# CSU-KangHu/HiTE

Hardware: AMD Instinct MI355X
Metric: candidate TE boundaries/sec on 1 Gbp synthetic genome (fine stage: copy finding+gather+align+vote+judge) (higher is better)
Workload: dtype u8; 1 GPU; C3: 1000 Mbp synthetic genome, 2500 TIR + 2500 LTR families, 50000 candidates/GPU judged as TIR (copy finding by minimizer-index lookup inside the timed step; index build 0.0 s untimed); genome_bp=1000000000, candidates_per_gpu=50000, candidate_bases=192511237, copies=799813, copy_table=found, is_te=34225, parallelism=replicated genome, candidates per rank x1, all-gather of 32-B calls

## Files before the change

### hite_amd/_lib.py

```python
import ctypes as C
import os

import numpy as np

_HERE = os.path.dirname(os.path.abspath(__file__))
SO_PATH = os.path.join(_HERE, "libhite_gpu.so")

HITE_TE = {"tir": 0, "helitron": 1, "non_ltr": 2}
INFO = {0: "", 1: "nb", 2: "fl1", 3: "EXC"}
HITE_SUBCLUSTER_CHUNK = 64


class HiteError(RuntimeError):
    pass


class HiteCall(C.Structure):
    _fields_ = [("is_te", C.c_int32), ("info", C.c_int32), ("row_num", C.c_int32), ("bstart", C.c_int32),
                ("bend", C.c_int32), ("cons_len", C.c_int32), ("cons_off", C.c_int64)]


CALL_DTYPE = np.dtype([("is_te", "<i4"), ("info", "<i4"), ("row_num", "<i4"), ("bstart", "<i4"), ("bend", "<i4"),
                       ("cons_len", "<i4"), ("cons_off", "<i8")])
assert CALL_DTYPE.itemsize == 32 and C.sizeof(HiteCall) == 32
LCV_DTYPE = np.dtype([("body", "<u8"), ("care", "<u8"), ("gap_min", "u1"), ("gap_max", "u1"), ("body_len", "u1"), ("pad", "u1", (5,))])
assert LCV_DTYPE.itemsize == 24
HELITRON_MAX_BODY, HELITRON_MAX_GAP = 32, 63

_lib = None


def load():
    global _lib
    if _lib is None:
        if not os.path.exists(SO_PATH):
            raise HiteError("libhite_gpu.so not built: run `python -c 'import __graft_entry__ as g; g.build()'` "
                            "(or make -C hite_amd/csrc); there is no CPU fallback")
        lib = C.CDLL(SO_PATH)
        lib.hite_last_error.restype = C.c_char_p
        lib.hite_genome_bases.restype = C.c_int64
        lib.hite_host_free.restype = None
        lib.hite_host_free.argtypes = [C.c_void_p]
        lib.hite_protein_lib_release.restype = None
        lib.hite_protein_lib_release.argtypes = [C.c_void_p]
        _lib = lib
    return _lib


def _p(a):
    return a.ctypes.data_as(C.c_void_p) if a is not None else None


def _arr(x, dtype):
    return np.ascontiguousarray(x, dtype=dtype)


def seed_sub_shard(rank, world, s, S):
    if world <= 1:
        rank, world = 0, 1
    return rank * S + s, world * S


class Context:

    def __init__(self, device=0):
        self.lib = load()
        h = C.c_void_p()
        rc = self.lib.hite_ctx_create(int(device), C.byref(h))
        if rc != 0:
            raise HiteError("hite_ctx_create(device=%d) failed: %d (no usable GPU?)" % (device, rc))
        self.h = h
        self.device = device

    def copy_config(self, aligned_interval):
        self._check(self.lib.hite_copy_config_ctx(self.h, -1 if aligned_interval is None else int(bool(aligned_interval))), "hite_copy_config_ctx")

    def release_copy_index(self):
        if getattr(self, "_copy_state", None) is not None and getattr(self, "h", None):
            self.lib.hite_copy_index_release(self._copy_state)
        self._copy_state = None

    def close(self):
        self.release_copy_index()
        for lib in list(getattr(self, "_prot_libs", ())):
            lib.release()
        if getattr(self, "_pipe_state", None) is not None and getattr(self, "h", None):
            self.lib.hite_pipeline_release(self._pipe_state)
            self._pipe_state = C.c_void_p(None)
        if getattr(self, "h", None):
            self.lib.hite_ctx_destroy(self.h)
            self.h = None

    def __del__(self):
        try:
            self.close()
        except Exception:
            pass

    def _check(self, rc, what):
        if rc != 0:
            msg = self.lib.hite_last_error(self.h)
            raise HiteError("%s failed: %d %s" % (what, rc, (msg or b"").decode(errors="replace")))

    def genome_pack(self, seqs):
        bs = [s.encode() if isinstance(s, str) else bytes(s) for s in seqs]
        off = np.zeros(len(bs) + 1, dtype=np.int64)
        np.cumsum([len(b) for b in bs], out=off[1:])
        buf = np.frombuffer(b"".join(bs), dtype=np.uint8)
        self._check(self.lib.hite_genome_pack(self.h, _p(buf), _p(off), len(bs)), "hite_genome_pack")
        self.contig_len = np.diff(off)

    def set_contig_order(self, names):
        if names is None:
            self._check(self.lib.hite_set_contig_order(self.h, None, 0), "hite_set_contig_order")
            return
        keyed = sorted(range(len(names)), key=lambda i: (names[i] + ":").encode())
        rank = np.zeros(len(names), dtype=np.int32)
        rank[keyed] = np.arange(len(names), dtype=np.int32)
        self._check(self.lib.hite_set_contig_order(self.h, _p(rank), len(names)), "hite_set_contig_order")

    def genome_pack_dev(self, d_ptr, contig_off, stream=0):
        off = _arr(contig_off, np.int64)
        self._check(self.lib.hite_genome_pack_dev(self.h, C.c_void_p(d_ptr), _p(off), len(off) - 1, C.c_void_p(stream)),
                    "hite_genome_pack_dev")
        self.contig_len = np.diff(off)

    def flank_gather(self, contig, start1, end1, minus, flank=50):
        n = len(contig)
# ... 926 lines not shown
```

### hite_amd/csrc/hite_common.h

```cpp
#pragma once
#include <hip/hip_runtime.h>
#include <stdint.h>
#include <stdio.h>
#include <string.h>
#include <stdlib.h>
#include "../../include/hite_gpu.h"

#define HITE_WAVE 64
#define HITE_BLOCK 256

#define JUDGE_CLS_BLOCK 0
#define JUDGE_CLS_WAVE 1
#define JUDGE_CLS_LDS 2
#define JUDGE_LDS_WAVE_SIZES 3
#define JUDGE_LDS_BLOCK_SIZES 2
#define JUDGE_NCLS (JUDGE_CLS_LDS + JUDGE_LDS_WAVE_SIZES + JUDGE_LDS_BLOCK_SIZES)
#define HITE_AUX_STREAMS (JUDGE_NCLS - 1)
struct JudgeFuse {
    const uint8_t *win;
    const int64_t *win_off;
    const int32_t *win_len;
    const int32_t *row_first;
    const int64_t *ops_base;
    const uint16_t *ops;
    const uint32_t *lay;
    const int32_t *last_extra;
    const int32_t *row_map;
    const int32_t *rows_eff;
};

struct hite_ctx {
    int device;
    char err[512];
    uint32_t *d_bases;
    uint32_t *d_nmask;
    int64_t *d_contig_off;
    int64_t *h_contig_off;
    int32_t n_contigs;
    int64_t n_bases;
    int64_t genome_epoch;
    int64_t *mask_log;
    int64_t mask_log_n, mask_log_cap;
    void *d_scratch;
    size_t scratch_bytes;
    void *d_scratch2;
    size_t scratch2_bytes;
    int prof_on;
    int prof_n;
    char prof_name[64][32];
    double prof_ms[64];
    int64_t prof_count[64];
    int prof_pending;
    void *prof_ev[512][2];
    int prof_stage[512];
    void *align_state;
    const int32_t *d_msa_row_map;
    const int32_t *d_msa_rows_eff;
    uint32_t *d_msa_lay;
    int msa_long;
    const int64_t *d_msa_win_off;
    const int32_t *d_msa_win_len;
    const uint32_t *d_msa_pads;
    int32_t copy_interval;
    int32_t *d_contig_rank;
    void *aux_stream[HITE_AUX_STREAMS];
    void *aux_fork;
    void *aux_join[HITE_AUX_STREAMS];
    int32_t seed_rank, seed_world;
    const uint8_t *d_judge_cls;
    JudgeFuse judge_fuse;
    void *fmea_arena;
    int32_t subcluster_chunk;
    int64_t subcluster_batch_bytes;
    int64_t framecluster_batch_bytes;
    int64_t pairhsp_batch_pairs;
    int64_t ltrscan_batch_bytes;
};
void hite_fmea_release(hite_ctx *ctx);
int hite_aux_streams(hite_ctx *ctx, int k, hipStream_t *st, hipEvent_t *fork_ev, hipEvent_t *join_ev);

int hite_prof_begin(hite_ctx *ctx, const char *name, hipStream_t st);
void hite_prof_end(hite_ctx *ctx, int token, hipStream_t st);
void hite_prof_resolve(hite_ctx *ctx);

#define HITE_CHECK(ctx, call)                                                                         \
    do {                                                                                              \
        hipError_t e__ = (call);                                                                      \
        if (e__ != hipSuccess) {                                                                      \
            if (ctx) snprintf((ctx)->err, sizeof((ctx)->err), "%s:%d %s: %s", __FILE__, __LINE__, #call, \
                              hipGetErrorString(e__));                                                \
            return HITE_EHIP;                                                                         \
        }                                                                                             \
    } while (0)

int hite_scratch_reserve(hite_ctx *ctx, size_t bytes, void **out);
int hite_scratch2_reserve(hite_ctx *ctx, size_t bytes, void **out);

__device__ __forceinline__ int lane_id() { return threadIdx.x & 63; }
__device__ __forceinline__ int wave_id() { return threadIdx.x >> 6; }

__device__ __forceinline__ int sym_class(uint8_t c) {
    switch (c) {
        case 'A': return 0;
        case 'C': return 1;
        case 'G': return 2;
        case 'T': return 3;
        case '-': return 5;
        default: return 4;
    }
}
__device__ __forceinline__ uint8_t class_sym(int k) { return (uint8_t)("ACGTN-"[k]); }
__device__ __forceinline__ uint8_t fold_sym(uint8_t c) { return class_sym(sym_class(c)); }
// ... 44 lines not shown
```

### hite_amd/csrc/hite_ctx.hip

```cpp
#include "hite_common.h"
#include "hite_hostbuf.h"
#include "hite_align.h"
#include "hite_genome.h"

extern "C" int hite_version(void) { return 1; }

extern "C" int hite_ctx_create(int device_id, hite_ctx **out) {
    if (!out) return HITE_EINVAL;
    int ndev = 0;
    if (hipGetDeviceCount(&ndev) != hipSuccess || ndev <= 0) return HITE_ENODEV;
    if (device_id < 0 || device_id >= ndev) return HITE_EINVAL;
    hite_ctx *c = (hite_ctx *)calloc(1, sizeof(hite_ctx));
    if (!c) return HITE_ENOMEM;
    c->device = device_id;
    c->copy_interval = -1;
    c->subcluster_chunk = HITE_SUBCLUSTER_CHUNK;
    if (const char *e = getenv("HITE_SUBCLUSTER_CHUNK_ROWS")) {
        const long v = strtol(e, nullptr, 10);
        if (v >= 1 && v <= HITE_SUBCLUSTER_CHUNK) c->subcluster_chunk = (int32_t)v;
    }
    if (const char *e = getenv("HITE_SUBCLUSTER_BATCH_BYTES")) {
        const long long v = strtoll(e, nullptr, 10);
        if (v >= 1) c->subcluster_batch_bytes = (int64_t)v;
    }
    if (const char *e = getenv("HITE_FRAMECLUSTER_BATCH_BYTES")) {
        const long long v = strtoll(e, nullptr, 10);
        if (v >= 1 && v <= ((long long)1 << 30)) c->framecluster_batch_bytes = (int64_t)v;
    }
    if (const char *e = getenv("HITE_PAIRHSP_BATCH_PAIRS")) {
        const long long v = strtoll(e, nullptr, 10);
        if (v >= 1 && v <= ((long long)1 << 24)) c->pairhsp_batch_pairs = (int64_t)v;
    }
    if (const char *e = getenv("HITE_LTRSCAN_BATCH_BYTES")) {
        const long long v = strtoll(e, nullptr, 10);
        if (v >= 1 && v <= ((long long)1 << 30)) c->ltrscan_batch_bytes = (int64_t)v;
    }
    if (hipSetDevice(device_id) != hipSuccess) { free(c); return HITE_EHIP; }
    *out = c;
    return HITE_OK;
}

static void free_genome(hite_ctx *c) {
    if (c->d_contig_rank) { (void)hipFree(c->d_contig_rank); c->d_contig_rank = nullptr; }
    if (c->d_bases) (void)hipFree(c->d_bases);
    if (c->d_nmask) (void)hipFree(c->d_nmask);
    if (c->d_contig_off) (void)hipFree(c->d_contig_off);
    free(c->h_contig_off);
    c->d_bases = c->d_nmask = nullptr;
    c->d_contig_off = nullptr;
    c->h_contig_off = nullptr;
    c->n_contigs = 0;
    c->n_bases = 0;
    c->genome_epoch++;
    c->mask_log_n = 0;
}

extern "C" void hite_ctx_destroy(hite_ctx *c) {
    if (!c) return;
    (void)hipSetDevice(c->device);
    free_genome(c);
    free(c->mask_log);
    hite_align_release(c);
    hite_fmea_release(c);
    if (c->d_scratch) (void)hipFree(c->d_scratch);
    if (c->d_scratch2) (void)hipFree(c->d_scratch2);
    if (c->d_contig_rank) (void)hipFree(c->d_contig_rank);
    if (c->aux_fork) (void)hipEventDestroy((hipEvent_t)c->aux_fork);
    for (int i = 0; i < HITE_AUX_STREAMS; i++) {
// ... 421 lines not shown
```

### hite_amd/csrc/hite_msa.hip

```cpp
#include "hite_common.h"
#include "hite_hostbuf.h"
#include "hite_align.h"
#include "hite_scan.h"
#include "hite_fill.h"

#define MSA_MAXR 128

struct MsaParams {
    int n;
    int64_t total_rows;
    const uint8_t *win;
    const int64_t *win_off;
    const int32_t *win_len;
    const int32_t *row_first;
    const int64_t *ops_base;
    uint16_t *ops;
    int32_t *cols_out;
    int32_t *status;
    const int32_t *row_map;
    const int32_t *rows_eff;
    const uint32_t *pads;
    uint32_t *lay;
};

__device__ __forceinline__ int msa_rows(const int32_t *__restrict__ rows_eff, const int32_t *__restrict__ row_first, int c) {
    return rows_eff ? rows_eff[c] : row_first[c + 1] - row_first[c];
}
__device__ __forceinline__ int msa_src(const int32_t *__restrict__ row_map, int64_t g0, int r) {
    return row_map ? row_map[g0 + r] - (int)g0 : r;
}

__device__ __forceinline__ int row_ins_s(const uint16_t *__restrict__ rop, int p, int m, int nrow, int start) {
    int prev_end = start;
    if (p > 0) { unsigned o = rop[p - 1]; prev_end = (int)(o & 0x7fff) + ((o >> 15) ? 0 : 1); }
    int q = p < m ? (int)(rop[p] & 0x7fff) : nrow;
    return q - prev_end;
}
__device__ __forceinline__ int row_ins(const uint16_t *__restrict__ rop, int p, int m, int nrow) {
    const unsigned o = rop[p - 1];
    const int prev_end = (int)(o & 0x7fff) + ((o >> 15) ? 0 : 1);
    int q = p < m ? (int)(rop[p] & 0x7fff) : nrow;
    return q - prev_end;
}

__global__ void __launch_bounds__(256) star_layout_kernel(MsaParams P) {
    __shared__ int s_scan[8];
    const int c = blockIdx.x;
    if (c >= P.n) return;
    const int64_t g0 = P.row_first[c];
    const int R = msa_rows(P.rows_eff, P.row_first, c);
    if (R <= 0) { if (threadIdx.x == 0) P.cols_out[c] = 0; return; }
    const int m = P.win_len[g0];
    uint16_t *ops = P.ops + P.ops_base[c];
    uint16_t *insmax = ops;
    uint16_t *bstart = ops + (int64_t)R * (m + 1);
    if (P.status[c]) { if (threadIdx.x == 0) P.cols_out[c] = 0; return; }
    int running = 0;
// ... 246 lines not shown
    }
};
template <int NU>
__global__ void __launch_bounds__(256) star_fill_sparse_kernel(FillSparseParams Q) {
    const FillParams &P = Q.F;
    const int c = blockIdx.x;
    if (c >= P.n) return;
    const int C = P.cols[c];
    if (C <= 0 || (Q.cls && Q.cls[c] >= JUDGE_CLS_LDS)) return;
    const int64_t g0 = P.row_first[c];
    const int R = msa_rows(P.rows_eff, P.row_first, c);
    const int m = P.win_len[g0];
    const uint16_t *ops = P.ops + P.ops_base[c];
    const uint32_t *lay = Q.lay + (P.ops_base[c] >> 1);
    const int le = Q.last_extra[c];
    uint8_t *out = P.msa + P.msa_off[c];
    const int rs = m + 1;
    int r = blockIdx.y;
    if (r >= R) return;
    __shared__ unsigned s_defer[FILL_DEFER_CAP];
    __shared__ int s_ndefer;
    if (threadIdx.x == 0) s_ndefer = 0;
    __syncthreads();
    const bool can_defer = R <= 0xffff && m < 0xffff;
    int src = msa_src(P.row_map, g0, r);
    int64_t woff = P.win_off[g0 + src];
    int nrow = P.win_len[g0 + src];
    while (r < R) {
        const int rn = r + (int)gridDim.y;
        int64_t woff_n = 0; int nrow_n = 0;
        if (rn < R) { const int sn = msa_src(P.row_map, g0, rn); woff_n = P.win_off[g0 + sn]; nrow_n = P.win_len[g0 + sn]; }
        const uint8_t *b = P.win + woff;
        const uint16_t *rop = ops + (int64_t)r * rs;
        uint8_t *row = out + (int64_t)r * C;
        if (can_defer) fill_sparse_row<uint8_t *, 256, NU, FillDefer>(row, b, nrow, rop, lay, m, le, r == 0 , (int)threadIdx.x,
                                                                      FillDefer{s_defer, &s_ndefer, (unsigned)r});
        else fill_sparse_row<uint8_t *, 256, NU>(row, b, nrow, rop, lay, m, le, r == 0, (int)threadIdx.x);
        r = rn; woff = woff_n; nrow = nrow_n;
    }
    __syncthreads();
    const int nd = s_ndefer < FILL_DEFER_CAP ? s_ndefer : FILL_DEFER_CAP;
    for (int i = threadIdx.x; i < nd; i += 256) {
        const int rr = (int)(s_defer[i] >> 16), p = (int)(s_defer[i] & 0xffffu);
        const int sr = msa_src(P.row_map, g0, rr);
        const uint8_t *b = P.win + P.win_off[g0 + sr];
        const int nr = P.win_len[g0 + sr];
        const uint16_t *rop = ops + (int64_t)rr * rs;
        const unsigned w = lay[p];
        const unsigned oc = rr == 0 ? (unsigned)p : (p < m ? (unsigned)rop[p] : 0x8000u);
        fill_sparse_block<uint8_t *>(out + (int64_t)rr * C, b, nr, rop, m, le, rr == 0, p, w, oc);
    }
}

__global__ void __launch_bounds__(256) msa_compact_rows_kernel(int n, const int32_t *__restrict__ row_first,
                                                               const int32_t *__restrict__ win_len, const int64_t *__restrict__ ops_base,
                                                               uint16_t *__restrict__ ops_all, const int32_t *__restrict__ cand_flag,
                                                               const int32_t *__restrict__ row_dead, int32_t *__restrict__ row_map,
                                                               int32_t *__restrict__ rows_eff) {
    const int c = blockIdx.x;
    if (c >= n) return;
    const int g0 = row_first[c], R = row_first[c + 1] - g0;
    if (R <= 0) { if (threadIdx.x == 0) rows_eff[c] = 0; return; }
    if (cand_flag[c] != 2) {
        for (int r = threadIdx.x; r < R; r += 256) row_map[g0 + r] = g0 + r;
        if (threadIdx.x == 0) rows_eff[c] = R;
        return;
    }
    const int m = win_len[g0];
    uint16_t *ops = ops_all + ops_base[c];
    int k = 0;
    for (int r = 0; r < R; r++) {
        if (row_dead[g0 + r]) continue;
        if (k != r) for (int p = threadIdx.x; p <= m; p += 256) ops[(int64_t)k * (m + 1) + p] = ops[(int64_t)r * (m + 1) + p];
        if (threadIdx.x == 0) row_map[g0 + k] = g0 + r;
        k++;
        __syncthreads();
    }
    if (threadIdx.x == 0) rows_eff[c] = k;
}
__global__ void msa_rows_out_kernel(int n, const int32_t *__restrict__ row_first, const int32_t *__restrict__ rows_eff,
                                    int32_t *__restrict__ rows_out) {
    const int c = blockIdx.x * blockDim.x + threadIdx.x;
    if (c < n) rows_out[c] = rows_eff ? rows_eff[c] : row_first[c + 1] - row_first[c];
}

__global__ void row_pad_scan_kernel(int64_t total_rows, const uint8_t *__restrict__ win, const int64_t *__restrict__ win_off,
                                    const int32_t *__restrict__ win_len, int32_t *__restrict__ len2, uint32_t *__restrict__ pads) {
    const int64_t g = (int64_t)blockIdx.x * blockDim.x + threadIdx.x;
    if (g >= total_rows) return;
    const uint8_t *b = win + win_off[g];
    const int n = win_len[g];
    int pf = 0, pb = 0;
    if (n > 0 && HITE_IS_ROW_PAD(b[0])) { pf = 1; while (pf < n && HITE_IS_ROW_PAD(b[pf])) pf++; }
    if (pf < n && HITE_IS_ROW_PAD(b[n - 1])) { pb = 1; while (pf + pb < n && HITE_IS_ROW_PAD(b[n - 1 - pb])) pb++; }
    len2[g] = n - pb;
    pads[g] = (uint32_t)pf | ((uint32_t)pb << 16);
}
__global__ void __launch_bounds__(256) ops_pad_fix_kernel(int n, const int32_t *__restrict__ row_first, const int32_t *__restrict__ win_len,
                                                          const int64_t *__restrict__ ops_base, uint16_t *__restrict__ ops_all,
                                                          const uint32_t *__restrict__ pads, const int32_t *__restrict__ row_map,
                                                          const int32_t *__restrict__ rows_eff, int32_t *__restrict__ len2) {
    const int c = blockIdx.x;
    if (c >= n) return;
    const int g0 = row_first[c];
    const int R = rows_eff ? rows_eff[c] : row_first[c + 1] - g0;
    if (R >= 1 && threadIdx.x == 0) len2[g0] = win_len[g0];
// ... 8 lines not shown
        uint16_t *o = ops + (int64_t)k * (m + 1);
        if (lane == 0) o[-1] = (uint16_t)(0x8000u | (unsigned)pf);
        if (pf) {
            for (int base = 0; base < m; base += 64) {
                const int p = base + lane;
                const bool hit = p < m && (int)(o[p < m ? p : 0] & 0x7fffu) < pf;
                if (hit) o[p] = (uint16_t)(0x8000u | (unsigned)pf);
                if (__ballot(hit) != ~0ull) break;
            }
        }
        if (pb) {
            for (int top = m; top > 0; top -= 64) {
                const int p = top - 1 - lane;
                const bool hit = p >= 0 && (int)(o[p >= 0 ? p : 0] & 0x7fffu) >= hi;
                if (hit) o[p] = (uint16_t)(0x8000u | (unsigned)hi);
                if (__ballot(hit) != ~0ull) break;
            }
        }
    }
}

static int star_msa_launch(hite_ctx *ctx, int32_t n, const uint8_t *d_win, const int64_t *d_win_off,
                           const int32_t *d_win_len, const int32_t *d_row_first, int64_t total_rows, const int64_t *d_ops_base,
                           int64_t ops_elems, int32_t max_win_len, int32_t *d_cols_out, int32_t *d_status,
                           int32_t *d_new_cols, int32_t *d_last_extra, int32_t *d_rows_out, int32_t *d_info, void *stream) {
    if (!ctx || n < 0 || total_rows < 0 || max_win_len <= 0 || max_win_len > 32767) return HITE_EINVAL;
    if (n == 0) return HITE_OK;
    const size_t ops_bytes = ((size_t)ops_elems * 2 + 255) & ~(size_t)255;
    const size_t rows_bytes = ((size_t)total_rows * 4 + 255) & ~(size_t)255, cand_bytes = ((size_t)n * 4 + 255) & ~(size_t)255;
    void *opsb = nullptr;
    const size_t lay_bytes = d_new_cols ? (((size_t)ops_elems / 2 + 32768 + 16) * 4 + 255) & ~(size_t)255 : 0;
    int rc = hite_scratch2_reserve(ctx, ops_bytes + 2 * rows_bytes + 2 * cand_bytes + lay_bytes + 2 * rows_bytes + 256, &opsb);
    if (rc) return rc;
    uint8_t *base = (uint8_t *)opsb;
    int32_t *row_dead = (int32_t *)(base + ops_bytes), *row_map = (int32_t *)(base + ops_bytes + rows_bytes);
    int32_t *rows_eff = (int32_t *)(base + ops_bytes + 2 * rows_bytes), *cand_flag = (int32_t *)(base + ops_bytes + 2 * rows_bytes + cand_bytes);
    hipStream_t st = (hipStream_t)stream;
    HITE_CHECK(ctx, hipMemsetAsync(d_status, 0, (size_t)n * 4, st));
    HITE_CHECK(ctx, hipMemsetAsync(cand_flag, 0, (size_t)n * 4, st));
    int64_t before[8], after[8];
    rc = hite_align_stats(ctx, before, 0);
    if (rc) return rc;
    rc = hite_align_run(ctx, n, d_win, d_win_off, d_win_len, d_row_first, total_rows, d_ops_base, (uint16_t *)opsb, row_dead, cand_flag, d_info,
                        max_win_len > 1000 ? "_long" : "_short", st);
    if (rc) return rc;
    rc = hite_align_stats(ctx, after, 0);
    if (rc) return rc;
    const bool dropped = after[4] > before[4];
    int32_t *len2 = (int32_t *)(base + ops_bytes + 2 * rows_bytes + 2 * cand_bytes + lay_bytes);
    uint32_t *pads = (uint32_t *)((uint8_t *)len2 + rows_bytes);
    if (total_rows > 0)
        hipLaunchKernelGGL(row_pad_scan_kernel, dim3((unsigned)((total_rows + 255) / 256)), dim3(256), 0, st, total_rows, d_win, d_win_off, d_win_len,
                           len2, pads);
    ctx->d_msa_win_off = d_win_off; ctx->d_msa_win_len = len2; ctx->d_msa_pads = pads; ctx->msa_long = max_win_len > 1536;
    MsaParams P;
    P.n = n; P.total_rows = total_rows; P.win = d_win; P.win_off = d_win_off; P.win_len = len2; P.row_first = d_row_first;
    P.ops_base = d_ops_base; P.ops = (uint16_t *)opsb; P.cols_out = d_cols_out; P.status = d_status;
    P.row_map = nullptr; P.rows_eff = nullptr; P.pads = pads;
    P.lay = d_new_cols ? (uint32_t *)(base + ops_bytes + 2 * rows_bytes + 2 * cand_bytes) : nullptr;
    ctx->d_msa_lay = P.lay;
    if (dropped) {
        hipLaunchKernelGGL(msa_compact_rows_kernel, dim3(n), dim3(256), 0, st, n, d_row_first, d_win_len, d_ops_base, (uint16_t *)opsb, cand_flag,
                           row_dead, row_map, rows_eff);
        P.row_map = row_map; P.rows_eff = rows_eff;
    }
    ctx->d_msa_row_map = P.row_map; ctx->d_msa_rows_eff = P.rows_eff;
    hipLaunchKernelGGL(ops_pad_fix_kernel, dim3(n), dim3(256), 0, st, n, d_row_first, d_win_len, d_ops_base, (uint16_t *)opsb, pads, P.row_map,
                       P.rows_eff, len2);
    if (d_rows_out) hipLaunchKernelGGL(msa_rows_out_kernel, dim3((n + 255) / 256), dim3(256), 0, st, n, d_row_first, P.rows_eff, d_rows_out);
    int tk;
    if (d_new_cols) {
        tk = hite_prof_begin(ctx, max_win_len > 1000 ? "star_layout_sparse_kernel_long" : "star_layout_sparse_kernel_short", st);
        hipLaunchKernelGGL(star_layout_sparse_kernel, dim3(n), dim3(256), 0, st, P, d_new_cols, d_last_extra);
    } else {
        tk = hite_prof_begin(ctx, "star_layout_kernel", st);
        hipLaunchKernelGGL(star_layout_kernel, dim3(n), dim3(256), 0, st, P);
    }
    hite_prof_end(ctx, tk, st);
    HITE_CHECK(ctx, hipGetLastError());
    return HITE_OK;
}

extern "C" int hite_star_msa_dev(hite_ctx *ctx, int32_t n, const uint8_t *d_win, const int64_t *d_win_off,
                                 const int32_t *d_win_len, const int32_t *d_row_first, int64_t total_rows, const int64_t *d_ops_base,
                                 int64_t ops_elems, int32_t max_win_len, int32_t *d_cols_out, int32_t *d_status,
                                 int32_t *d_rows_out, void *stream) {
    return star_msa_launch(ctx, n, d_win, d_win_off, d_win_len, d_row_first, total_rows, d_ops_base, ops_elems, max_win_len,
                           d_cols_out, d_status, nullptr, nullptr, d_rows_out, nullptr, stream);
}

extern "C" int hite_star_msa_sparse_dev(hite_ctx *ctx, int32_t n, const uint8_t *d_win, const int64_t *d_win_off,
                                        const int32_t *d_win_len, const int32_t *d_row_first, int64_t total_rows,
                                        const int64_t *d_ops_base, int64_t ops_elems, int32_t max_win_len, int32_t *d_cols_out,
                                        int32_t *d_status, int32_t *d_new_cols, int32_t *d_last_extra, int32_t *d_rows_out,
                                        void *stream) {
    if (!d_new_cols || !d_last_extra) return HITE_EINVAL;
    return star_msa_launch(ctx, n, d_win, d_win_off, d_win_len, d_row_first, total_rows, d_ops_base, ops_elems, max_win_len,
                           d_cols_out, d_status, d_new_cols, d_last_extra, d_rows_out, nullptr, stream);
}

extern "C" int hite_star_msa_fill_sparse_dev(hite_ctx *ctx, int32_t n, const uint8_t *d_win, const int64_t *d_win_off,
                                             const int32_t *d_win_len, const int32_t *d_row_first, const int64_t *d_ops_base,
                                             const int32_t *d_new_cols, const int32_t *d_last_extra, const int64_t *d_msa_off,
                                             uint8_t *d_msa, void *stream) {
    if (!ctx || n < 0 || !ctx->d_scratch2 || !d_new_cols || !d_last_extra) return HITE_EINVAL;
    if (n == 0) return HITE_OK;
    FillSparseParams Q;
    FillParams &P = Q.F;
    P.n = n; P.win = d_win; P.win_off = ctx->d_msa_win_off ? ctx->d_msa_win_off : d_win_off; P.win_len = ctx->d_msa_win_len ? ctx->d_msa_win_len : d_win_len;
    P.row_first = d_row_first; P.ops_base = d_ops_base;
    P.ops = (const uint16_t *)ctx->d_scratch2; P.cols = d_new_cols; P.msa_off = d_msa_off; P.msa = d_msa;
    P.row_map = ctx->d_msa_row_map; P.rows_eff = ctx->d_msa_rows_eff; P.pads = ctx->d_msa_pads;
    Q.last_extra = d_last_extra; Q.lay = ctx->d_msa_lay;
    Q.cls = ctx->judge_fuse.win ? ctx->d_judge_cls : nullptr;
    if (!Q.lay) return HITE_EINVAL;
#ifndef FILL_U_LONG
#define FILL_U_LONG 8
#endif
#ifndef FILL_U_SHORT
#define FILL_U_SHORT 4
#endif
    if (ctx->msa_long) hipLaunchKernelGGL(HIP_KERNEL_NAME(star_fill_sparse_kernel<FILL_U_LONG>), dim3(n, 4), dim3(256), 0, (hipStream_t)stream, Q);
    else hipLaunchKernelGGL(HIP_KERNEL_NAME(star_fill_sparse_kernel<FILL_U_SHORT>), dim3(n, 4), dim3(256), 0, (hipStream_t)stream, Q);
    HITE_CHECK(ctx, hipGetLastError());
    return HITE_OK;
}

extern "C" int hite_star_msa_fill_dev(hite_ctx *ctx, int32_t n, const uint8_t *d_win, const int64_t *d_win_off,
                                      const int32_t *d_win_len, const int32_t *d_row_first, const int64_t *d_ops_base, const int32_t *d_cols,
                                      const int64_t *d_msa_off, uint8_t *d_msa, void *stream) {
    if (!ctx || n < 0 || !ctx->d_scratch2) return HITE_EINVAL;
    if (n == 0) return HITE_OK;
    FillParams P;
    P.n = n; P.win = d_win; P.win_off = ctx->d_msa_win_off ? ctx->d_msa_win_off : d_win_off; P.win_len = ctx->d_msa_win_len ? ctx->d_msa_win_len : d_win_len;
    P.row_first = d_row_first; P.ops_base = d_ops_base;
    P.ops = (const uint16_t *)ctx->d_scratch2; P.cols = d_cols; P.msa_off = d_msa_off; P.msa = d_msa;
    P.row_map = ctx->d_msa_row_map; P.rows_eff = ctx->d_msa_rows_eff; P.pads = ctx->d_msa_pads;
    hipLaunchKernelGGL(star_fill_kernel, dim3(n, 4), dim3(256), 0, (hipStream_t)stream, P);
    HITE_CHECK(ctx, hipGetLastError());
    return HITE_OK;
}

static int star_msa_host(hite_ctx *ctx, int32_t n, const uint8_t *win, const int64_t *win_off,
                         const int32_t *row_first, int32_t *cols_out, int32_t *rows_out, int64_t msa_cap, uint8_t *msa_out,
                         int64_t *msa_off_out, int32_t *info_out, bool sparse, uint8_t **msa_alloc = nullptr, int64_t *msa_bytes = nullptr) try {
    if (!ctx || n < 0 || !win || !win_off || !row_first || !cols_out) return HITE_EINVAL;
    if (n == 0) return HITE_OK;
    HITE_CHECK(ctx, hipSetDevice(ctx->device));
    int64_t total_rows = row_first[n];
    std::vector<int64_t> ops_base((size_t)n + 1);
    int64_t acc = 0;
    int maxlen = 1;
    for (int c = 0; c < n; c++) {
        int R = row_first[c + 1] - row_first[c];
        if (R <= 0) return HITE_EINVAL;
        int64_t m = win_off[row_first[c] + 1] - win_off[row_first[c]];
        ops_base[c] = acc;
        acc += (int64_t)(R + 1) * (m + 1);
        for (int r = 0; r < R; r++) {
            int64_t L = win_off[row_first[c] + r + 1] - win_off[row_first[c] + r];
            if (L <= 0 || L > 32767) return HITE_EINVAL;
            if (L > maxlen) maxlen = (int)L;
        }
    }
    ops_base[n] = acc;
    DevBuf dw, dwo, dwl, drf, dob, dcols, dst, dmo, dmsa, dnew, dlast, drows, dinfo;
    hipError_t e;
    {
        std::vector<int32_t> wl((size_t)total_rows + 1);
        std::vector<int64_t> wo((size_t)total_rows + 1);
        int64_t pos = 0;
        for (int64_t g = 0; g < total_rows; g++) { wl[g] = (int32_t)(win_off[g + 1] - win_off[g]); wo[g] = pos; pos += ((int64_t)wl[g] + 15) & ~(int64_t)15; }
        wo[total_rows] = pos;
        std::vector<uint8_t> wpad((size_t)pos + 16, 0);
        for (int64_t g = 0; g < total_rows; g++) memcpy(wpad.data() + wo[g], win + win_off[g], (size_t)wl[g]);
// ... 75 lines not shown
```

### include/hite_gpu.h

```cpp
#ifndef HITE_GPU_H
#define HITE_GPU_H
#include <stdint.h>

#ifdef __cplusplus
extern "C" {
#endif

#define HITE_ROW_PAD 0x2e
#define HITE_IS_ROW_PAD(c) (((c) & 0x20u) != 0)

#define HITE_OK 0
#define HITE_EINVAL (-1)
#define HITE_ENOMEM (-2)
#define HITE_EHIP (-3)
#define HITE_ECAP (-4)
#define HITE_ENODEV (-5)

#define HITE_TE_TIR 0
#define HITE_TE_HELITRON 1
#define HITE_TE_NON_LTR 2

#define HITE_INFO_NONE 0
#define HITE_INFO_NB 1
#define HITE_INFO_FL1 2
// ... 207 lines not shown
void hite_copy_index_release(void *state);
int hite_copy_stats(void *state, int64_t out[4]);
int hite_copy_stats_ext(void *state, int64_t out[8]);

int hite_seed_allvsall_dev(hite_ctx *ctx, void **state_io, int64_t seg_len, int64_t max_anchors, int32_t **d_qseg, int32_t **d_sseg,
                           int64_t **d_qs, int64_t **d_qe, int64_t **d_ss, int64_t **d_se, int64_t *n_out, int64_t *stats_out);
int hite_seed_segments(hite_ctx *ctx, int64_t seg_len, int32_t cap, int32_t *seg_chrom, int64_t *seg_off, int32_t *nseg_out);
int hite_seed_shard(hite_ctx *ctx, int32_t rank, int32_t world);
int hite_seed_allvsall(hite_ctx *ctx, void **state_io, int64_t seg_len, int64_t max_anchors, int64_t cap, int32_t *qseg,
                       int32_t *sseg, int64_t *qs, int64_t *qe, int64_t *ss, int64_t *se, int64_t *n_out, int64_t *stats_out);
int hite_find_copies(hite_ctx *ctx, void **state_io, int32_t n_cand, const uint8_t *cand, const int64_t *cand_off,
                     int64_t cap, int32_t *copy_first, int32_t *contig, int64_t *start1, int64_t *end1, uint8_t *minus,
                     int32_t *anchors, int64_t *n_out);
int hite_find_copies_dev(hite_ctx *ctx, void *state, int32_t n_cand, const uint8_t *d_cand, const int64_t *d_cand_off,
                         int64_t cand_bytes, int32_t **d_copy_first, int64_t *n_copies, int32_t **d_contig,
                         int64_t **d_start1, int64_t **d_end1, uint8_t **d_minus, int32_t **d_anchors, void *stream);
int hite_find_copies_restricted_dev(hite_ctx *ctx, void **state_io, int32_t n_cand, const uint8_t *d_cand, const int64_t *d_cand_off,
                                    int64_t cand_bytes, int32_t **d_copy_first, int64_t *n_copies, int32_t **d_contig,
                                    int64_t **d_start1, int64_t **d_end1, uint8_t **d_minus, int32_t **d_anchors, void *stream);
int hite_find_copies_restricted(hite_ctx *ctx, void **state_io, int32_t n_cand, const uint8_t *cand, const int64_t *cand_off,
                                int64_t cap, int32_t *copy_first, int32_t *contig, int64_t *start1, int64_t *end1, uint8_t *minus,
                                int32_t *anchors, int64_t *n_out);
int hite_copy_clips_dev(void *state, const uint32_t **d_clip, int64_t *n);
int hite_copy_clips(void *state, int64_t cap, uint32_t *clip);

int hite_align_config(hite_ctx *ctx, int32_t exact_cap);
int hite_align_lanes(hite_ctx *ctx, int32_t min_cols);
int hite_align_stats(hite_ctx *ctx, int64_t *out8, int32_t reset);
int hite_star_msa(hite_ctx *ctx, int32_t n, const uint8_t *win, const int64_t *win_off, const int32_t *row_first,
                  int32_t *cols_out, int32_t *rows_out, int64_t msa_cap, uint8_t *msa_out, int64_t *msa_off_out);
int hite_star_msa_sparse(hite_ctx *ctx, int32_t n, const uint8_t *win, const int64_t *win_off, const int32_t *row_first,
                         int32_t *cols_out, int32_t *rows_out, int64_t msa_cap, uint8_t *msa_out, int64_t *msa_off_out);
int hite_star_msa_info(hite_ctx *ctx, int32_t n, const uint8_t *win, const int64_t *win_off, const int32_t *row_first,
                       int32_t *cols_out, int32_t *rows_out, int32_t *info_out, int64_t msa_cap, uint8_t *msa_out,
                       int64_t *msa_off_out);
int hite_star_msa_once(hite_ctx *ctx, int32_t n, const uint8_t *win, const int64_t *win_off, const int32_t *row_first,
                       int32_t sparse, int32_t *cols_out, int32_t *rows_out, int32_t *info_out, uint8_t **msa_out,
                       int64_t *msa_off_out, int64_t *msa_bytes_out);
void hite_host_free(void *p);
int hite_star_msa_dev(hite_ctx *ctx, int32_t n, const uint8_t *d_win, const int64_t *d_win_off,
                      const int32_t *d_win_len, const int32_t *d_row_first, int64_t total_rows, const int64_t *d_ops_base, int64_t ops_elems,
                      int32_t max_win_len, int32_t *d_cols_out, int32_t *d_status, int32_t *d_rows_out, void *stream);
int hite_star_msa_fill_dev(hite_ctx *ctx, int32_t n, const uint8_t *d_win, const int64_t *d_win_off,
                           const int32_t *d_win_len, const int32_t *d_row_first, const int64_t *d_ops_base, const int32_t *d_cols,
                           const int64_t *d_msa_off, uint8_t *d_msa, void *stream);
int hite_star_msa_sparse_dev(hite_ctx *ctx, int32_t n, const uint8_t *d_win, const int64_t *d_win_off,
                             const int32_t *d_win_len, const int32_t *d_row_first, int64_t total_rows,
                             const int64_t *d_ops_base, int64_t ops_elems, int32_t max_win_len, int32_t *d_cols_out,
                             int32_t *d_status, int32_t *d_new_cols, int32_t *d_last_extra, int32_t *d_rows_out, void *stream);
int hite_star_msa_fill_sparse_dev(hite_ctx *ctx, int32_t n, const uint8_t *d_win, const int64_t *d_win_off,
                                  const int32_t *d_win_len, const int32_t *d_row_first, const int64_t *d_ops_base,
                                  const int32_t *d_new_cols, const int32_t *d_last_extra, const int64_t *d_msa_off,
                                  uint8_t *d_msa, void *stream);

int hite_flank_region_align(hite_ctx *ctx, int32_t te_type, int32_t plant, int32_t n_cand, const uint8_t *cand,
                            const int64_t *cand_off, const int32_t *copy_first, int64_t n_copies, const int32_t *contig,
                            const int64_t *start1, const int64_t *end1, const uint8_t *minus, int32_t flank,
                            hite_call *calls, uint8_t *cons, int64_t cons_cap, int64_t *stats_out);
int hite_flank_region_align_dev(hite_ctx *ctx, void **state_io, int32_t te_type, int32_t plant, int32_t n_cand,
                                const uint8_t *d_cand, const int64_t *d_cand_off, const int32_t *d_copy_first,
                                int64_t n_copies, const int32_t *d_contig, const int64_t *d_start1, const int64_t *d_end1,
                                const uint8_t *d_minus, int32_t flank, hite_call *d_calls, uint8_t *d_cons,
                                int64_t cons_cap, int64_t *stats_out, void *stream);
int hite_clip_probe(hite_ctx *ctx, int32_t n_cand, const uint8_t *cand, const int64_t *cand_off, const int32_t *copy_first,
                    int64_t n_copies, const int32_t *contig, const int64_t *start1, const int64_t *end1, const uint8_t *minus,
                    uint32_t *clip_out);
int hite_fine_rows(hite_ctx *ctx, int32_t n_cand, const uint8_t *cand, const int64_t *cand_off, const int32_t *copy_first,
                   int64_t n_copies, const int32_t *contig, const int64_t *start1, const int64_t *end1, const uint8_t *minus,
                   const uint32_t *clip, int32_t flank, int32_t pass, int32_t *nrows, int64_t row_cap, int32_t *row_copy,
                   int32_t *row_len, uint8_t *row_trunc, int64_t *win_off, int64_t win_cap, uint8_t *win, int64_t *totals);
int hite_flank_region_align_clip(hite_ctx *ctx, int32_t te_type, int32_t plant, int32_t n_cand, const uint8_t *cand,
                                 const int64_t *cand_off, const int32_t *copy_first, int64_t n_copies, const int32_t *contig,
                                 const int64_t *start1, const int64_t *end1, const uint8_t *minus, const uint32_t *clip, int32_t flank,
                                 hite_call *calls, uint8_t *cons, int64_t cons_cap, int64_t *stats_out);
int hite_flank_region_align_clip_dev(hite_ctx *ctx, void **state_io, int32_t te_type, int32_t plant, int32_t n_cand,
                                     const uint8_t *d_cand, const int64_t *d_cand_off, const int32_t *d_copy_first,
                                     int64_t n_copies, const int32_t *d_contig, const int64_t *d_start1, const int64_t *d_end1,
                                     const uint8_t *d_minus, const uint32_t *d_clip, int32_t flank, hite_call *d_calls,
                                     uint8_t *d_cons, int64_t cons_cap, int64_t *stats_out, void *stream);
void hite_pipeline_release(void *state);

int hite_profile_enable(hite_ctx *ctx, int on);
int hite_profile_reset(hite_ctx *ctx);
int hite_profile_count(hite_ctx *ctx);
int hite_profile_get(hite_ctx *ctx, int idx, char *name_out, double *ms_total, int64_t *launches);

int hite_memcpy_d2h(void *dst, const void *d_src, int64_t bytes);

int hite_event_create(void **ev);
int hite_event_record(void *ev, void *stream);
int hite_event_elapsed_ms(void *ev_start, void *ev_stop, float *ms);
int hite_event_destroy(void *ev);

int hite_allgather_records(hite_ctx *ctx, void *nccl_comm, const void *d_send, void *d_recv, int64_t bytes_per_rank, void *stream);

#ifdef __cplusplus
}
#endif
#endif
```

Before: 679,800 candidates/s.

## Add LDS-tiled sparse MSA fill kernel with staged window loads and vector stores

Adds a new star-MSA sparse fill kernel that splits each MSA into column tiles of 512 positions, one wave per row. Each wave stages its source window in LDS with 16-byte loads and assembles the output row tile in LDS before writing it out with aligned 16-byte stores. Loads for the next row's ops and window are software-pipelined against the current row, and rows whose window doesn't fit the LDS slot fall back to a direct per-cell path. It is on by default (disable with HITE_FILL_TILES=0). It trades extra LDS traffic and wave syncs for coalesced global memory access, and is meant to replace the scattered byte writes of the old per-cell fill.

```diff
diff --git a/hite_amd/_lib.py b/hite_amd/_lib.py
--- a/hite_amd/_lib.py
+++ b/hite_amd/_lib.py
@@ -74,6 +74,14 @@
 
     def copy_config(self, aligned_interval):
         self._check(self.lib.hite_copy_config_ctx(self.h, -1 if aligned_interval is None else int(bool(aligned_interval))), "hite_copy_config_ctx")
+
+    def fill_config(self, tiles):
+        self._check(self.lib.hite_fill_config_ctx(self.h, -1 if tiles is None else int(bool(tiles))), "hite_fill_config_ctx")
+
+    def fill_tile_limits(self):
+        out = (C.c_int32 * 4)()
+        self._check(self.lib.hite_fill_tile_limits(out), "hite_fill_tile_limits")
+        return tuple(out)
 
     def release_copy_index(self):
         if getattr(self, "_copy_state", None) is not None and getattr(self, "h", None):
diff --git a/hite_amd/csrc/hite_common.h b/hite_amd/csrc/hite_common.h
--- a/hite_amd/csrc/hite_common.h
+++ b/hite_amd/csrc/hite_common.h
@@ -58,6 +58,8 @@
     const int32_t *d_msa_rows_eff;
     uint32_t *d_msa_lay;
     int msa_long;
+    int msa_max_len;
+    int32_t fill_tiles;
     const int64_t *d_msa_win_off;
     const int32_t *d_msa_win_len;
     const uint32_t *d_msa_pads;
diff --git a/hite_amd/csrc/hite_ctx.hip b/hite_amd/csrc/hite_ctx.hip
--- a/hite_amd/csrc/hite_ctx.hip
+++ b/hite_amd/csrc/hite_ctx.hip
@@ -14,6 +14,7 @@
     if (!c) return HITE_ENOMEM;
     c->device = device_id;
     c->copy_interval = -1;
+    c->fill_tiles = -1;
     c->subcluster_chunk = HITE_SUBCLUSTER_CHUNK;
     if (const char *e = getenv("HITE_SUBCLUSTER_CHUNK_ROWS")) {
         const long v = strtol(e, nullptr, 10);
diff --git a/hite_amd/csrc/hite_fill_tile.h b/hite_amd/csrc/hite_fill_tile.h
--- /dev/null
+++ b/hite_amd/csrc/hite_fill_tile.h
@@ -0,0 +1,125 @@
+#pragma once
+#include "hite_fill.h"
+
+#ifndef FT_NP
+#define FT_NP 8
+#endif
+#define FT_T (64 * FT_NP)
+#define FT_CH (FT_NP / 8)
+#define FT_LDS (1024 * FT_CH)
+#define FT_SLOT (FT_LDS - 16)
+#ifndef FT_ROWS
+#define FT_ROWS 1
+#endif
+
+typedef uint32_t FtV16 __attribute__((vector_size(16)));
+
+struct FtOps {
+    uint32_t o2[FT_NP / 2];
+    uint32_t oprev;
+};
+__device__ __forceinline__ unsigned ft_lane_op(const FtOps &L, int u) {
+    uint32_t o = L.o2[0] & 0xffffu;
+#pragma unroll
+    for (int x = 1; x < FT_NP; x++)
+        if (u == x) o = (L.o2[x >> 1] >> (16 * (x & 1))) & 0xffffu;
+    return o;
+}
+__device__ __forceinline__ int ft_end(unsigned o) { return (int)(o & 0x7fffu) + ((o >> 15) ? 0 : 1); }
+__device__ __forceinline__ unsigned ft_op(unsigned raw, int p, int m, int nrow, bool centre) {
+    if (p >= m) return 0x8000u | (unsigned)nrow;
+    return centre ? (unsigned)p : raw;
+}
+__device__ __forceinline__ unsigned ft_prev(unsigned raw, int p, bool centre) {
+    return centre ? (p == 0 ? 0x8000u : (unsigned)(p - 1)) : raw;
+}
+__device__ __forceinline__ FtOps ft_ops_load(const uint16_t *__restrict__ rop, int p0, int m, bool centre, bool first) {
+    FtOps L;
+#pragma unroll
+    for (int i = 0; i < FT_NP / 2; i++) L.o2[i] = 0;
+    L.oprev = 0;
+    if (centre) return L;
+    const int pc = p0 < m ? p0 : m;
+    uint32_t t[FT_NP / 2];
+    __builtin_memcpy(t, rop + pc, 2 * FT_NP);
+#pragma unroll
+    for (int i = 0; i < FT_NP / 2; i++) L.o2[i] = t[i];
+    L.oprev = rop[first && pc == 0 ? 0 : pc - 1];
+    return L;
+}
+__device__ __forceinline__ bool ft_row_plan(unsigned tprev, unsigned tlast, int P0, int pl, int m, int nrow, bool centre, int *qa, int *len) {
+    const int a = ft_end(ft_prev(tprev, P0, centre));
+    const int end = ft_end(ft_op(tlast, pl, m, nrow, centre));
+    *qa = a; *len = end - a;
+    return a >= 0 && end >= a && end <= nrow && end - a <= FT_SLOT;
+}
+__device__ __forceinline__ bool ft_tile_plan(unsigned wfirst, unsigned wnext, bool last_tile, int C, int *c0, int *W) {
+    *c0 = (int)(wfirst >> 16);
+    *W = (last_tile ? C : (int)(wnext >> 16)) - *c0;
+    return *W >= 0 && *W <= FT_SLOT;
+}
+__device__ __forceinline__ int ft_win_shift(const uint8_t *b, int qa) { return (int)((uintptr_t)(b + qa) & 15u); }
+__device__ __forceinline__ int ft_win_chunks(int sh, int len) { return (sh + len + 15) >> 4; }
+__device__ __forceinline__ void ft_win_load(FtV16 *v, const uint8_t *__restrict__ b, int qa, int len, int lane) {
+    const int sh = ft_win_shift(b, qa);
+    const FtV16 *src = (const FtV16 *)(b + qa - sh);
+    const int nch = ft_win_chunks(sh, len);
+#pragma unroll
+    for (int k = 0; k < FT_CH; k++) v[k] = src[lane + 64 * k < nch ? lane + 64 * k : 0];
+}
+template <class Lds>
+__device__ __forceinline__ void ft_win_put(Lds slot, const FtV16 *v, int nch, int lane) {
+#pragma unroll
+    for (int k = 0; k < FT_CH; k++)
+        if (lane + 64 * k < nch) ((FtV16 *)slot)[lane + 64 * k] = v[k];
+}
+template <class Lds>
+__device__ __forceinline__ void ft_cells(Lds img, Lds slot, const FtOps &L, const uint32_t *w, int p0, int m, int nrow, int le, bool centre,
+                                         int wb, int bias) {
+    unsigned rare = 0;
+#pragma unroll
+    for (int u = 0; u < FT_NP; u++) {
+        const int p = p0 + u;
+        const unsigned o = ft_op((L.o2[u >> 1] >> (16 * (u & 1))) & 0xffffu, p, m, nrow, centre);
+        const unsigned kw = w[u] & 0x7fffu;
+        const bool keep = (w[u] >> 15) & 1u, base = keep && !(o >> 15);
+        const uint8_t cb = slot[base ? wb + (int)(o & 0x7fffu) : 0];
+        if (keep) img[bias + (int)(w[u] >> 16) + (int)kw] = base ? cb : (uint8_t)'-';
+        if (p <= m && (kw != 0u || (p == m && le >= 0))) rare |= 1u << u;
+    }
+    while (rare) {
+        const int u = __builtin_ctz(rare);
+        rare &= rare - 1;
+        uint32_t wu = w[0], ou = L.o2[0] & 0xffffu, pu = L.oprev;
+#pragma unroll
+        for (int x = 1; x < FT_NP; x++)
+            if (u == x) { wu = w[x]; ou = (L.o2[x >> 1] >> (16 * (x & 1))) & 0xffffu; pu = (L.o2[(x - 1) >> 1] >> (16 * ((x - 1) & 1))) & 0xffffu; }
+        const int p = p0 + u;
+        const unsigned o = ft_op(ou, p, m, nrow, centre), op = ft_prev(pu, p, centre);
+        const int kw = (int)(wu & 0x7fffu), bs = bias + (int)(wu >> 16);
+        const int rp = ft_end(op), ins = (int)(o & 0x7fffu) - rp;
+        for (int k = 0; k < kw; k++) img[bs + k] = k < ins ? slot[wb + rp + k] : (uint8_t)'-';
+        if (p == m && le >= 0) img[bs + kw] = le < ins ? slot[wb + rp + le] : (uint8_t)'-';
+    }
+}
+__device__ __forceinline__ int ft_img_shift(const uint8_t *dst) { return (int)((uintptr_t)dst & 15u); }
+template <class Lds>
+__device__ __forceinline__ void ft_store(uint8_t *__restrict__ dst, Lds img, int W, int lane) {
+    const int a = ft_img_shift(dst);
+    const int head = min(W, (16 - a) & 15), nmid = (W - head) >> 4, tail = W - head - 16 * nmid;
+    if (lane < head) dst[lane] = img[a + lane];
+    FtV16 *d16 = (FtV16 *)(dst + head);
+#pragma unroll
+    for (int k = 0; k < FT_CH; k++)
+        if (lane + 64 * k < nmid) d16[lane + 64 * k] = ((const FtV16 *)(img + a + head))[lane + 64 * k];
+    if (lane < tail) dst[head + 16 * nmid + lane] = img[a + head + 16 * nmid + lane];
+}
+__device__ __forceinline__ void ft_cells_direct(uint8_t *row, const uint8_t *__restrict__ b, int nrow, const uint16_t *__restrict__ rop,
+                                                const uint32_t *__restrict__ lay, int m, int le, bool centre, int pa, int pb, int lane) {
+    for (int p = pa + lane; p < pb; p += 64) {
+        const unsigned w = lay[p];
+        const unsigned oc = centre ? (unsigned)p : (p < m ? (unsigned)rop[p] : 0x8000u);
+        if ((w >> 15) & 1u) row[(w >> 16) + (w & 0x7fffu)] = (oc >> 15) ? (uint8_t)'-' : b[oc & 0x7fffu];
+        fill_sparse_block<uint8_t *>(row, b, nrow, rop, m, le, centre, p, w, oc);
+    }
+}
diff --git a/hite_amd/csrc/hite_msa.hip b/hite_amd/csrc/hite_msa.hip
--- a/hite_amd/csrc/hite_msa.hip
+++ b/hite_amd/csrc/hite_msa.hip
@@ -3,6 +3,7 @@
 #include "hite_align.h"
 #include "hite_scan.h"
 #include "hite_fill.h"
+#include "hite_fill_tile.h"
 
 #define MSA_MAXR 128
 
@@ -355,6 +356,113 @@
     }
 }
 
+#ifndef FT_GRID_Z
+#define FT_GRID_Z 1
+#endif
+#define FT_WAVE_SYNC() do { __builtin_amdgcn_fence(__ATOMIC_ACQ_REL, "wavefront"); __builtin_amdgcn_wave_barrier(); } while (0)
+__global__ void __launch_bounds__(64 * FT_ROWS) star_fill_tile_kernel(FillSparseParams Q) {
+    const FillParams &P = Q.F;
+    const int c = blockIdx.x;
+    if (c >= P.n) return;
+    const int C = P.cols[c];
+    if (C <= 0 || (Q.cls && Q.cls[c] >= JUDGE_CLS_LDS)) return;
+    const int64_t g0 = P.row_first[c];
+    const int m = P.win_len[g0];
+    const int P0 = (int)blockIdx.y * FT_T;
+    if (P0 > m) return;
+    const int R = msa_rows(P.rows_eff, P.row_first, c);
+    const int lane = (int)threadIdx.x & 63, wave = __builtin_amdgcn_readfirstlane((int)threadIdx.x >> 6);
+    const int step = FT_ROWS * (int)gridDim.z;
+    int r = (int)blockIdx.z * FT_ROWS + wave;
+    if (r >= R) return;
+    const uint16_t *ops = P.ops + P.ops_base[c];
+    const uint32_t *lay = Q.lay + (P.ops_base[c] >> 1);
+    const int le = Q.last_extra[c];
+    uint8_t *out = P.msa + P.msa_off[c];
+    const int64_t rs = m + 1;
+    const int pl = min(P0 + FT_T - 1, m);
+    const int p0 = P0 + lane * FT_NP;
+    uint32_t w[FT_NP];
+#pragma unroll
+    for (int u = 0; u < FT_NP; u++) {
+        const int p = p0 + u;
+        const uint32_t wl = lay[p <= m ? p : m];
+        w[u] = p <= m ? wl : 0u;
+    }
+    int c0, W;
+    const bool tile_ok = ft_tile_plan(lay[P0], lay[pl < m ? pl + 1 : m], pl == m, C, &c0, &W);
+    __shared__ FtV16 s_slot[FT_ROWS][FT_LDS / 16], s_img[FT_ROWS][FT_LDS / 16];
+    uint8_t *slot = (uint8_t *)s_slot[wave], *img = (uint8_t *)s_img[wave];
+
+    int Rc = 0;
+  for (; r < R; ) {
+    Rc = min(R, r + 64 * step);
+    FtOps S0 = ft_ops_load(ops + r * rs, p0, m, r == 0, r == 0), S1, S2 = {};
+    S1 = ft_ops_load(ops + min(r + step, Rc - 1) * rs, p0, m, false, min(r + step, Rc - 1) == 0);
+    int64_t my_off = 0;
+    int my_len = 0;
+    if (r + lane * step < R) { const int s = msa_src(P.row_map, g0, r + lane * step); my_off = P.win_off[g0 + s]; my_len = P.win_len[g0 + s]; }
+    struct RowWin { const uint8_t *b; int n; };
+    auto row_win = [&](int i) -> RowWin {
+        const unsigned lo = (unsigned)__builtin_amdgcn_readlane((int)(my_off & 0xffffffff), i), hi = (unsigned)__builtin_amdgcn_readlane((int)(my_off >> 32), i);
+        return RowWin{P.win + (int64_t)(((uint64_t)hi << 32) | lo), __builtin_amdgcn_readlane(my_len, i)};
+    };
+    struct RowPlan { const uint8_t *b; int n, qa, len; bool ok; };
+    auto plan_row = [&](const FtOps &L, int i, int rr, FtV16 *v) -> RowPlan {
+        RowPlan pr;
+        const RowWin rw = row_win(i);
+        pr.b = rw.b; pr.n = rw.n;
+        const unsigned tprev = (unsigned)__builtin_amdgcn_readfirstlane((int)L.oprev);
+        const unsigned tlast = (unsigned)__builtin_amdgcn_readlane((int)ft_lane_op(L, (pl - P0) % FT_NP), (pl - P0) / FT_NP);
+        const bool ok = ft_row_plan(tprev, tlast, P0, pl, m, pr.n, rr == 0, &pr.qa, &pr.len) && tile_ok;
+        pr.ok = __builtin_amdgcn_readfirstlane((int)ok) != 0; pr.qa = __builtin_amdgcn_readfirstlane(pr.qa); pr.len = __builtin_amdgcn_readfirstlane(pr.len);
+        ft_win_load(v, pr.b, pr.ok ? pr.qa : 0, pr.ok ? pr.len : 0, lane);
+        return pr;
+    };
+    int i = 0;
+    const int rbase = r;
+    unsigned long long bad = 0;
+    RowPlan pa, pb = {};
+    auto step_row = [&](FtOps &A, FtOps &B, FtOps &N, FtV16 *vA, FtV16 *vB) -> bool {
+        const int rn = r + step, rnn = rn + step;
+        N = ft_ops_load(ops + min(rnn, Rc - 1) * rs, p0, m, false, min(rnn, Rc - 1) == 0);
+        pb = plan_row(B, min(i + 1, 63), min(rn, Rc - 1), vB);
+        uint8_t *row = out + (int64_t)r * C;
+        if (pa.ok) {
+            const int sh = ft_win_shift(pa.b, pa.qa);
+            ft_win_put(slot, vA, ft_win_chunks(sh, pa.len), lane);
+            FT_WAVE_SYNC();
+            ft_cells(img, slot, A, w, p0, m, pa.n, le, r == 0, sh - pa.qa, ft_img_shift(row + c0) - c0);
+            FT_WAVE_SYNC();
+            ft_store(row + c0, img, W, lane);
+            FT_WAVE_SYNC();
+        } else {
+            bad |= 1ull << i;
+        }
+        pa = pb; r = rn; i++;
+        return r < Rc;
+    };
+    FtV16 V0[FT_CH], V1[FT_CH];
+#pragma unroll
+    for (int k = 0; k < FT_CH; k++) V0[k] = V1[k] = FtV16{0, 0, 0, 0};
+    pa = plan_row(S0, 0, r, V0);
+    for (;;) {
+        if (!step_row(S0, S1, S2, V0, V1)) break;
+        if (!step_row(S1, S2, S0, V1, V0)) break;
+        if (!step_row(S2, S0, S1, V0, V1)) break;
+        if (!step_row(S0, S1, S2, V1, V0)) break;
+        if (!step_row(S1, S2, S0, V0, V1)) break;
+        if (!step_row(S2, S0, S1, V1, V0)) break;
+    }
+    while (bad) {
+        const int k = __builtin_ctzll(bad), rr = rbase + k * step;
+        bad &= bad - 1;
+        const RowWin rw = row_win(k);
+        ft_cells_direct(out + (int64_t)rr * C, rw.b, rw.n, ops + rr * rs, lay, m, le, rr == 0, P0, pl + 1, lane);
+    }
+  }
+}
+
 __global__ void __launch_bounds__(256) msa_compact_rows_kernel(int n, const int32_t *__restrict__ row_first,
                                                                const int32_t *__restrict__ win_len, const int64_t *__restrict__ ops_base,
                                                                uint16_t *__restrict__ ops_all, const int32_t *__restrict__ cand_flag,
@@ -469,7 +577,7 @@
     if (total_rows > 0)
         hipLaunchKernelGGL(row_pad_scan_kernel, dim3((unsigned)((total_rows + 255) / 256)), dim3(256), 0, st, total_rows, d_win, d_win_off, d_win_len,
                            len2, pads);
-    ctx->d_msa_win_off = d_win_off; ctx->d_msa_win_len = len2; ctx->d_msa_pads = pads; ctx->msa_long = max_win_len > 1536;
+    ctx->d_msa_win_off = d_win_off; ctx->d_msa_win_len = len2; ctx->d_msa_pads = pads; ctx->msa_long = max_win_len > 1536; ctx->msa_max_len = max_win_len;
     MsaParams P;
     P.n = n; P.total_rows = total_rows; P.win = d_win; P.win_off = d_win_off; P.win_len = len2; P.row_first = d_row_first;
     P.ops_base = d_ops_base; P.ops = (uint16_t *)opsb; P.cols_out = d_cols_out; P.status = d_status;
@@ -514,6 +622,28 @@
     if (!d_new_cols || !d_last_extra) return HITE_EINVAL;
     return star_msa_launch(ctx, n, d_win, d_win_off, d_win_len, d_row_first, total_rows, d_ops_base, ops_elems, max_win_len,
                            d_cols_out, d_status, d_new_cols, d_last_extra, d_rows_out, nullptr, stream);
+}
+
+static int g_fill_tiles = -1;
+static int fill_tiles_mode(const hite_ctx *ctx) {
+    if (ctx->fill_tiles >= 0) return ctx->fill_tiles;
+    int v = __atomic_load_n(&g_fill_tiles, __ATOMIC_RELAXED);
+    if (v < 0) {
+        const char *e = getenv("HITE_FILL_TILES");
+        v = (e && !strcmp(e, "0")) ? 0 : 1;
+        __atomic_store_n(&g_fill_tiles, v, __ATOMIC_RELAXED);
+    }
+    return v;
+}
+extern "C" int hite_fill_config_ctx(hite_ctx *ctx, int32_t mode) {
+    if (!ctx || mode < -1 || mode > 1) return HITE_EINVAL;
+    ctx->fill_tiles = mode;
+    return HITE_OK;
+}
+extern "C" int hite_fill_tile_limits(int32_t out[4]) {
+    if (!out) return HITE_EINVAL;
+    out[0] = FT_T; out[1] = FT_SLOT; out[2] = FT_ROWS; out[3] = FT_GRID_Z;
+    return HITE_OK;
 }
 
 extern "C" int hite_star_msa_fill_sparse_dev(hite_ctx *ctx, int32_t n, const uint8_t *d_win, const int64_t *d_win_off,
@@ -537,7 +667,9 @@
 #ifndef FILL_U_SHORT
 #define FILL_U_SHORT 4
 #endif
-    if (ctx->msa_long) hipLaunchKernelGGL(HIP_KERNEL_NAME(star_fill_sparse_kernel<FILL_U_LONG>), dim3(n, 4), dim3(256), 0, (hipStream_t)stream, Q);
+    if (fill_tiles_mode(ctx) && ctx->msa_max_len > 0)
+        hipLaunchKernelGGL(star_fill_tile_kernel, dim3(n, ctx->msa_max_len / FT_T + 1, FT_GRID_Z), dim3(64 * FT_ROWS), 0, (hipStream_t)stream, Q);
+    else if (ctx->msa_long) hipLaunchKernelGGL(HIP_KERNEL_NAME(star_fill_sparse_kernel<FILL_U_LONG>), dim3(n, 4), dim3(256), 0, (hipStream_t)stream, Q);
     else hipLaunchKernelGGL(HIP_KERNEL_NAME(star_fill_sparse_kernel<FILL_U_SHORT>), dim3(n, 4), dim3(256), 0, (hipStream_t)stream, Q);
     HITE_CHECK(ctx, hipGetLastError());
     return HITE_OK;
diff --git a/include/hite_gpu.h b/include/hite_gpu.h
--- a/include/hite_gpu.h
+++ b/include/hite_gpu.h
@@ -283,6 +283,8 @@
                                   const int32_t *d_win_len, const int32_t *d_row_first, const int64_t *d_ops_base,
                                   const int32_t *d_new_cols, const int32_t *d_last_extra, const int64_t *d_msa_off,
                                   uint8_t *d_msa, void *stream);
+int hite_fill_config_ctx(hite_ctx *ctx, int32_t mode);
+int hite_fill_tile_limits(int32_t out[4]);
 
 int hite_flank_region_align(hite_ctx *ctx, int32_t te_type, int32_t plant, int32_t n_cand, const uint8_t *cand,
                             const int64_t *cand_off, const int32_t *copy_first, int64_t n_copies, const int32_t *contig,
```

Measured after the change: 703,700 candidates/s (median of 6 runs). 3.5% higher.
